# haidar-farhat/NU_Scaler

Hardware: AMD Instinct MI355X
Metric: Mpixels/sec (in+out) at 1080p→4K ×2 upscale + interp, 1/2/4/8 GPU (higher is better)
Workload: dtype u8 frames, f32 taps

## Files before the change

nu_scaler_amd/csrc/nus_host.cpp:

```cpp
#include "nus_host.hpp"

#include <condition_variable>
#include <thread>

#include "nus_copy.hpp"
#include "nus_host_util.hpp"

#include <cstdarg>
#include <cstdio>
#include <cstring>

namespace nus {


HipUpscaler::HipUpscaler(Quality q, Algorithm a) : quality_(q), algorithm_(a) {}

HipUpscaler::~HipUpscaler() { release(); }

const char *HipUpscaler::name() const
{
    switch (algorithm_) {
    case Algorithm::Bilinear: return "WgpuBilinearUpscaler";
    case Algorithm::Lanczos3: return "HipLanczos3Upscaler";
    case Algorithm::Bicubic: return "HipBicubicUpscaler";
// ... 564 lines not shown

uint32_t HipUpscaler::band_alignment(uint32_t n_frames) const
{
    switch (variant_) {
    case Variant::LanczosX2RegWin: return lanczos_x2_rows_per_wave(n_frames, false);
    case Variant::NearestX2:
    case Variant::BilinearX2Int: return 4;
    default: return 0;
    }
}

int HipUpscaler::enqueue(const uint8_t *d_in, uint8_t *d_out, uint32_t n_frames, hipStream_t stream, const BlendSrc *blend,
                         const UnitDst *unit, uint32_t row0, uint32_t rows)
{
    UpscaleLaunch L;
    L.in = d_in;
    L.out = d_out;
    L.row0 = row0;
    L.rows = rows;
    L.iw = iw_;
    L.ih = ih_;
    L.ow = ow_;
    L.oh = oh_;
    L.n_frames = n_frames;
    L.stream = stream;
    L.in_sel = input_selector(in_format_);
    if (blend) {
        L.in_stride = blend->a_stride;
        L.in_b = blend->b;
        L.in_b_stride = blend->b_stride;
        L.blend_t = blend->t;
    }
    hipEvent_t ev_begin = nullptr, ev_end = nullptr;
    if (profiling_) {
        if (prof_used_ + 2 > prof_events_.size()) {
            for (int i = 0; i < 64; ++i) {
                hipEvent_t ev;
                NUS_HIP(hipEventCreate(&ev));
                prof_events_.push_back(ev);
            }
        }
        ev_begin = prof_events_[prof_used_];
        ev_end = prof_events_[prof_used_ + 1];
        prof_used_ += 2;
        NUS_HIP(hipEventRecord(ev_begin, stream));
    }
    constexpr uint32_t kEdgeBesideMinFrames = 8;
    const bool beside = variant_ == Variant::LanczosX2RegWin && edge_stream_ && s_edge_ && ev_fork_ && ev_join_ &&
                        n_frames >= kEdgeBesideMinFrames;
    if (beside) {
        NUS_HIP(hipEventRecord(ev_fork_, stream));
        NUS_HIP(hipStreamWaitEvent(s_edge_, ev_fork_, 0));
    }
    hipError_t e = hipSuccess;
    switch (variant_) {
    case Variant::NearestTable: e = launch_nearest_table(L, dt_); break;
    case Variant::NearestX2: e = launch_nearest_x2(L); break;
    case Variant::NearestRatio: e = launch_nearest_ratio(L); break;
    case Variant::BilinearTable: e = launch_bilinear_table(L, dt_, wgsl_bilinear_); break;
    case Variant::BilinearX2Int: e = launch_bilinear_x2_int(L); break;
    case Variant::BilinearRatio: e = launch_bilinear_ratio(L, dt_); break;
    case Variant::LanczosGeneral: e = launch_lanczos_general(L, dt_, lanczos_exact_, 0); break;
    case Variant::ResizeWin:
        e = launch_resize_win(L, dt_, lanczos_exact_, resize_ncols_max_, resize_union_taps_, win_outputs_per_lane_);
        break;
    case Variant::ResizeRows:
        e = launch_resize_rows(L, dt_, lanczos_exact_, resize_ncols_max_, resize_small_taps_, resize_union_taps_);
        break;
    case Variant::ResizeDown: e = launch_resize_down(L, dt_, lanczos_exact_, resize_ncols_max_, tx_.lz_max_taps, down_seg_w_); break;
    case Variant::FsrEasu: e = launch_fsr1(L, 0, easu_sharpness(), rcas_sharpness(), fsr_fast_); break;
    case Variant::FsrRcas: e = launch_fsr1(L, 1, easu_sharpness(), rcas_sharpness()); break;
    case Variant::Fsr1Fused: e = launch_fsr1(L, 2, easu_sharpness(), rcas_sharpness(), fsr_fast_); break;
    case Variant::Fsr1TwoPass: {
        if (fsr_pending_) e = hipStreamWaitEvent(stream, ev_fsr_, 0);
        const size_t in_frame = (size_t)iw_ * ih_ * 4, out_frame = (size_t)ow_ * oh_ * 4;
        for (uint32_t done = 0; done < n_frames && e == hipSuccess; done += kFsrScratchFrames) {
            const uint32_t m = n_frames - done < kFsrScratchFrames ? n_frames - done : kFsrScratchFrames;
            UpscaleLaunch E = L;
            E.in = L.in + (size_t)done * in_frame;
            E.out = fsr_scratch_;
            E.n_frames = m;
            e = launch_fsr1(E, 0, easu_sharpness(), rcas_sharpness(), fsr_fast_);
            if (e != hipSuccess) break;
            UpscaleLaunch Rc = L;
            Rc.in = fsr_scratch_;
            Rc.out = L.out + (size_t)done * out_frame;
            Rc.iw = ow_, Rc.ih = oh_;
            Rc.n_frames = m;
            Rc.in_sel = kSelRGBA;
            e = launch_fsr1(Rc, 1, easu_sharpness(), rcas_sharpness());
        }
        if (e == hipSuccess) e = hipEventRecord(ev_fsr_, stream);
        fsr_pending_ = e == hipSuccess;
        break;
    }
    case Variant::LanczosR43RegWin: {
        uint32_t th = rows_per_wave_;
        if (th == 0) {
            const uint64_t rows_total = (uint64_t)ih_ * ((iw_ + 185) / 186) * n_frames;
            uint64_t t = rows_total / 12288;
            t = t < 12 ? 12 : (t > 36 ? 36 : t);
            const uint64_t blocks = (ih_ + t - 1) / t;
            th = (uint32_t)(((ih_ + blocks - 1) / blocks + 2) / 3 * 3);
        }
        e = launch_lanczos_r43(L, dt_, lanczos_exact_, th);
        if (e == hipSuccess) e = launch_lanczos_r43_edges(L, dt_, lanczos_exact_);
        break;
    }
    case Variant::LanczosPqRegWin: {
        uint32_t th = rows_per_wave_;
        if (th == 0) {
            const uint32_t cols = lanczos_pq_strip_cols(pq_p_, pq_q_);
            const uint64_t rows_total = (uint64_t)ih_ * ((iw_ + cols - 1) / cols) * n_frames;
            uint64_t t = rows_total / 12288;
            t = t < 12 ? 12 : (t > 36 ? 36 : t);
            const uint64_t blocks = (ih_ + t - 1) / t;
            th = (uint32_t)(((ih_ + blocks - 1) / blocks + pq_q_ - 1) / pq_q_ * pq_q_);
        }
        if (lanczos_exact_ && pq_exact_fallback_)
            e = launch_resize_win(L, dt_, true, resize_ncols_max_, resize_union_taps_, win_outputs_per_lane_);
        else
            e = launch_lanczos_pq(L, dt_, lanczos_exact_, pq_p_, pq_q_, th, pq_narrow_ && pq_narrow_allowed_);
        break;
    }
    case Variant::LanczosR32RegWin: {
        uint32_t th = rows_per_wave_;
        if (th == 0) {
            const uint64_t rows_total = (uint64_t)ih_ * ((iw_ + 239) / 240) * n_frames;
            uint64_t t = rows_total / 12288;
            t = t < 12 ? 12 : (t > 48 ? 48 : t);
            const uint64_t blocks = (ih_ + t - 1) / t;
            th = (uint32_t)((ih_ + blocks - 1) / blocks + 1) & ~1u;
        }
        e = launch_lanczos_r32(L, dt_, lanczos_exact_, th);
        if (e == hipSuccess) e = launch_lanczos_r32_edges(L, dt_, lanczos_exact_);
        break;
    }
    case Variant::LanczosXsRegWin:
    {
        uint32_t th = rows_per_wave_;
        if (th == 0) {
            const uint64_t rows_total = (uint64_t)ih_ * ((iw_ + kLanczosX2StripCols - 1) / kLanczosX2StripCols) * n_frames;
            uint64_t t = rows_total / 16384;
            t = t < 8 ? 8 : (t > 16 ? 16 : t);
            const uint64_t blocks = (ih_ + t - 1) / t;
            th = (uint32_t)((ih_ + blocks - 1) / blocks);
        }
        e = launch_lanczos_xs(L, dt_, lanczos_exact_, xs_factor_, th);
        if (e == hipSuccess) e = launch_lanczos_xs_edges(L, dt_, lanczos_exact_, xs_factor_);
        break;
    }
    case Variant::LanczosX2RegWin: {
        {
            const hipStream_t es = beside ? s_edge_ : stream;
            UpscaleLaunch E = L;
            E.stream = es;
            if (unit) {
                UpscaleLaunch R = E;
                R.in_b = nullptr;
                e = launch_lanczos_x2_edges(R, dt_, lanczos_exact_);
                if (e != hipSuccess) return fail_hip(e, "kernel launch");
                E.out = unit->out_mid;
            }
            e = launch_lanczos_x2_edges(E, dt_, lanczos_exact_);
            if (e != hipSuccess) return fail_hip(e, "kernel launch");
            if (beside) NUS_HIP(hipEventRecord(ev_join_, s_edge_));
        }
        const uint32_t th = lanczos_x2_rows_per_wave(n_frames, unit != nullptr);
        if (unit) {
            UnitOutputs U;
            U.out_mid = unit->out_mid;
            U.mid = unit->mid;
            U.order = unit_order_;
            e = launch_lanczos_x2_unit(L, dt_, lanczos_exact_, th, U);
        } else {
            e = launch_lanczos_x2(L, dt_, lanczos_exact_, th);
        }
        break;
    }
    }
    if (e != hipSuccess) {
        if (beside) (void)hipStreamSynchronize(s_edge_);
        return fail_hip(e, "kernel launch");
    }
    if (beside) NUS_HIP(hipStreamWaitEvent(stream, ev_join_, 0));
    if (ev_end) NUS_HIP(hipEventRecord(ev_end, stream));
    return kOk;
}

int HipUpscaler::set_profiling(bool on)
{
    std::lock_guard<std::mutex> lk(mu_);
    profiling_ = on;
    return kOk;
}

int HipUpscaler::profile_collect(uint64_t *launches, double *total_ms)
{
    std::lock_guard<std::mutex> lk(mu_);
    double sum = 0.0;
    if (prof_used_) NUS_HIP(hipSetDevice(device_));
    for (size_t i = 0; i + 1 < prof_used_; i += 2) {
        NUS_HIP(hipEventSynchronize(prof_events_[i + 1]));
        float ms = 0.0f;
        NUS_HIP(hipEventElapsedTime(&ms, prof_events_[i], prof_events_[i + 1]));
        sum += ms;
    }
    if (launches) *launches = prof_used_ / 2;
    if (total_ms) *total_ms = sum;
    prof_used_ = 0;
    return kOk;
}

int HipUpscaler::upscale_device(const void *d_in, void *d_out, uint32_t n_frames, hipStream_t stream)
{
    std::lock_guard<std::mutex> lk(mu_);
    if (!initialized_) return fail(kNotInitialized, "Upscaler not initialized. Call initialize() first.");
    if (!d_in || !d_out) return fail(kInvalidArgument, "upscale_device: null device pointer");
    if (n_frames == 0) return kOk;
    if ((reinterpret_cast<uintptr_t>(d_in) % 16) || (reinterpret_cast<uintptr_t>(d_out) % 16))
        return fail(kInvalidArgument, "upscale_device: device pointers must be 16-byte aligned");
    if (n_frames > 1 && (((size_t)iw_ * ih_ * 4) % 16 || ((size_t)ow_ * oh_ * 4) % 16))
        return fail(kInvalidArgument, "upscale_device: batched frames need frame sizes that are multiples of 16 bytes");
    NUS_HIP(hipSetDevice(device_));
    return enqueue(static_cast<const uint8_t *>(d_in), static_cast<uint8_t *>(d_out), n_frames, stream);
}

int HipUpscaler::upscale_blend_device(const void *d_a, size_t a_stride, const void *d_b, size_t b_stride, float t,
                                      void *d_out, uint32_t n_frames, hipStream_t stream)
{
    std::lock_guard<std::mutex> lk(mu_);
    if (!initialized_) return fail(kNotInitialized, "Upscaler not initialized. Call initialize() first.");
    if (variant_ != Variant::LanczosX2RegWin)
        return fail(kUnsupported, "upscale_blend_device: only the exact-x2 resize kernels fuse the blend; "
                                  "run interpolate + upscale separately for this configuration");
    if (!d_a || !d_b || !d_out) return fail(kInvalidArgument, "upscale_blend_device: null device pointer");
    if (n_frames == 0) return kOk;
    if ((reinterpret_cast<uintptr_t>(d_a) % 16) || (reinterpret_cast<uintptr_t>(d_b) % 16) ||
        (reinterpret_cast<uintptr_t>(d_out) % 16) || (a_stride % 16) || (b_stride % 16) ||
        (n_frames > 1 && ((size_t)ow_ * oh_ * 4) % 16))
        return fail(kInvalidArgument, "upscale_blend_device: pointers and strides must be 16-byte aligned");
    NUS_HIP(hipSetDevice(device_));
    BlendSrc bs;
    bs.b = static_cast<const uint8_t *>(d_b);
    bs.a_stride = a_stride;
    bs.b_stride = b_stride;
    bs.t = t;
    return enqueue(static_cast<const uint8_t *>(d_a), static_cast<uint8_t *>(d_out), n_frames, stream, &bs);
}

int HipUpscaler::upscale_unit_device(const void *d_a, size_t a_stride, const void *d_b, size_t b_stride, float t, void *d_mid,
                                     void *d_out_real, void *d_out_mid, uint32_t n_units, hipStream_t stream)
{
    std::lock_guard<std::mutex> lk(mu_);
    if (!initialized_) return fail(kNotInitialized, "Upscaler not initialized. Call initialize() first.");
    if (variant_ != Variant::LanczosX2RegWin)
        return fail(kUnsupported, "upscale_unit_device: only the exact-x2 resize kernels run the whole step in one launch; "
                                  "run interpolate + upscale separately for this configuration");
    if (!d_a || !d_b || !d_out_real || !d_out_mid) return fail(kInvalidArgument, "upscale_unit_device: null device pointer");
    if (!(t >= 0.0f && t <= 1.0f)) return fail(kInvalidArgument, "upscale_unit_device: t must be in [0, 1]");
    if (n_units == 0) return kOk;
    auto misaligned = [](const void *p) { return (reinterpret_cast<uintptr_t>(p) % 16) != 0; };
    if (misaligned(d_a) || misaligned(d_b) || misaligned(d_mid) || misaligned(d_out_real) || misaligned(d_out_mid) ||
        (a_stride % 16) || (b_stride % 16) ||
        (n_units > 1 && (((size_t)ow_ * oh_ * 4) % 16 || ((size_t)iw_ * ih_ * 4) % 16)))
        return fail(kInvalidArgument, "upscale_unit_device: pointers, strides and frame sizes must be multiples of 16 bytes");
    const size_t in_bytes = (size_t)iw_ * ih_ * 4;
    if ((a_stride && a_stride < in_bytes) || (b_stride && b_stride < in_bytes))
        return fail(kInvalidArgument, "upscale_unit_device: frame stride smaller than a frame");
    NUS_HIP(hipSetDevice(device_));
    BlendSrc bs;
    bs.b = static_cast<const uint8_t *>(d_b);
    bs.a_stride = a_stride ? a_stride : in_bytes;
    bs.b_stride = b_stride ? b_stride : in_bytes;
    bs.t = t;
    UnitDst ud;
    ud.out_mid = static_cast<uint8_t *>(d_out_mid);
    ud.mid = static_cast<uint8_t *>(d_mid);
    return enqueue(static_cast<const uint8_t *>(d_a), static_cast<uint8_t *>(d_out_real), n_units, stream, &bs, &ud);
}

int HipUpscaler::upscale(const uint8_t *in, size_t in_len, uint8_t *out, size_t out_cap)
{
    const uint8_t *ins[1] = {in};
    const size_t lens[1] = {in_len};
    uint8_t *outs[1] = {out};
    return upscale_batch(ins, lens, 1, outs, out_cap);
}

int HipUpscaler::ensure_streams()
{
    if (s_in_ && s_k_ && s_out_) return kOk;
    if (!s_in_) NUS_HIP(hipStreamCreateWithFlags(&s_in_, hipStreamNonBlocking));
    if (!s_k_) NUS_HIP(hipStreamCreateWithFlags(&s_k_, hipStreamNonBlocking));
    if (!s_out_) NUS_HIP(hipStreamCreateWithFlags(&s_out_, hipStreamNonBlocking));
    return kOk;
}

int HipUpscaler::ensure_slot(Slot &S, size_t in_bytes, size_t out_bytes)
{
    if (S.d_in) return kOk;
    auto make = [&]() -> int {
        NUS_HIP(hipEventCreate(&S.k_begin));
        NUS_HIP(hipEventCreate(&S.k_end));
        NUS_HIP(hipEventCreateWithFlags(&S.in_done, hipEventDisableTiming));
        NUS_HIP(hipEventCreateWithFlags(&S.out_done, hipEventDisableTiming));
        for (hipEvent_t &ev : S.chunk_done) NUS_HIP(hipEventCreateWithFlags(&ev, hipEventDisableTiming));
        for (hipEvent_t &ev : S.band_in) NUS_HIP(hipEventCreateWithFlags(&ev, hipEventDisableTiming));
        for (hipEvent_t &ev : S.band_k) NUS_HIP(hipEventCreateWithFlags(&ev, hipEventDisableTiming));
        NUS_HIP(pinned_alloc(reinterpret_cast<void **>(&S.h_in), in_bytes));
        NUS_HIP(pinned_alloc(reinterpret_cast<void **>(&S.h_out), out_bytes));
        NUS_HIP(hipMalloc(reinterpret_cast<void **>(&S.d_out), out_bytes));
        NUS_HIP(hipMalloc(reinterpret_cast<void **>(&S.d_in), in_bytes));
        return kOk;
    };
    const int rc = make();
    if (rc != kOk) release_slot(S);
// ... 497 lines not shown
```

nu_scaler_amd/csrc/nus_k_lanczos_x2.hip:

```cpp

#ifndef NUS_STORE_AUX
#define NUS_STORE_AUX 2
#endif
#include "nus_device.hpp"

namespace nus {

namespace {

struct LanczosX2Args {
    const uint8_t *in;
    const uint8_t *in_b;
    float t;
    uint32_t sel;
    uint8_t *out;
    const float *wy6;
    float wxe[6];
    float wxo[6];
    uint32_t iw, ih;
    uint32_t nstrips, nrowblocks, th;
    size_t in_frame_bytes, in_b_frame_bytes, out_frame_bytes;
    uint8_t *out_mid;
    uint8_t *mid;
    uint32_t nframes, order;
// ... 455 lines not shown
        }
        role = in_grp / A.nstrips;
        strip = in_grp % A.nstrips;
    } else {
        frame = vid / gridDim.x;
        const uint32_t wave = __builtin_amdgcn_readfirstlane((vid % gridDim.x) * 4 + (threadIdx.x >> 6));
        if (wave >= A.nstrips * A.nrowblocks) return;
        strip = wave % A.nstrips;
        rb = wave / A.nstrips + A.rb0;
    }
    const int c = (int)(strip * kLanczosX2StripCols) - 4 + lane * 4;
    int cl = c < 0 ? 0 : c;
    cl = cl > (int)A.iw - 4 ? (int)A.iw - 4 : cl;
    const uint8_t *src = A.in + (size_t)frame * A.in_frame_bytes;
    const uint8_t *src_b = BLEND ? A.in_b + (size_t)frame * A.in_b_frame_bytes : src;
    float t = A.t;
    uint8_t *out = A.out;
    MidStore ms;
    if constexpr (UNIT) {
        const bool real = role == 0;
        src_b = real ? src : src_b;
        t = real ? 0.0f : t;
        out = real ? A.out : A.out_mid;
        const bool owner = lane >= 1 && lane <= (int)(kLanczosX2StripCols / 4) && c >= 0 && c + 4 <= (int)A.iw;
        ms.lane_off = owner ? (uint32_t)c * 4u : 0x80000000u;
        ms.rs = __builtin_amdgcn_make_buffer_rsrc(A.mid + (size_t)frame * ((size_t)A.iw * A.ih * 4u), 0,
                                                  real || A.mid == nullptr ? 0u : A.iw * A.ih * 4u, 0x00020000);
    } else {
        ms.lane_off = 0;
        ms.rs = __builtin_amdgcn_make_buffer_rsrc(nullptr, 0, 0, 0x00020000);
    }
    const __amdgpu_buffer_rsrc_t rs = __builtin_amdgcn_make_buffer_rsrc(
        out + (size_t)frame * A.out_frame_bytes, 0, (uint32_t)A.out_frame_bytes, 0x00020000);
#ifndef NUS_LZ_ALIGNED_STORES
#define NUS_LZ_ALIGNED_STORES 1
#endif
#ifndef NUS_LZ_MAIN_WRITES_EDGES
#define NUS_LZ_MAIN_WRITES_EDGES 0
#endif
    auto computes_stored_pixels = [&](int L) {
        const int cc = (int)(strip * kLanczosX2StripCols) - 4 + L * 4;
#if NUS_LZ_ALIGNED_STORES && NUS_LZ_MAIN_WRITES_EDGES
        return L >= 1 && L <= (int)(kLanczosX2StripCols / 4) && cc >= 0 && cc + 4 <= (int)A.iw;
#else
        return L >= 1 && L <= (int)(kLanczosX2StripCols / 4) && cc >= 4 && cc + 8 <= (int)A.iw;
#endif
    };
    constexpr bool SWAP = lanczos_x2_swap_stores(EXACT, NARROW), LDSX = lanczos_x2_lds_exchange(EXACT, NARROW);
    RowStore st;
    st.lane = lane;
#if NUS_LZ_CONTIG_STORES
    if constexpr (SWAP) {
        const int span0 = ((int)(strip * kLanczosX2StripCols) - 4) * 8;
        const int la = lane < 32 ? lane : lane - 32, lb = lane < 32 ? lane + 32 : lane;
        const int half = lane < 32 ? 0 : 16;
        st.off_a = computes_stored_pixels(la) ? (uint32_t)(span0 + 32 * la + half) : 0x80000000u;
        st.off_b = computes_stored_pixels(lb) ? (uint32_t)(span0 + 32 * lb + half) : 0x80000000u;
        st.idx_a = st.idx_b = 0;
    } else {
        constexpr int SKIP = NUS_LZ_ALIGNED_STORES ? 32 : 0;
        const int span0 = ((int)(strip * kLanczosX2StripCols) - 4) * 8;
        const int pa = SKIP + 16 * lane, pb = SKIP + 1024 + 16 * lane;
        st.idx_a = pa / 16;
        st.idx_b = pb / 16 < 128 ? pb / 16 : 127;
        st.off_a = computes_stored_pixels(pa / 32) ? (uint32_t)(span0 + pa) : 0x80000000u;
        st.off_b = pb / 32 < 64 && computes_stored_pixels(pb / 32) ? (uint32_t)(span0 + pb) : 0x80000000u;
    }
#else
    st.off_a = computes_stored_pixels(lane) ? (uint32_t)c * 8u : 0x80000000u;
    st.off_b = st.off_a + 16u;
    st.idx_a = st.idx_b = 0;
#endif
    const uint32_t in_off = (uint32_t)cl * 4u;
    const int r0 = (int)(rb * A.th);
    const int r_end = (r0 + (int)A.th) < (int)A.ih ? (r0 + (int)A.th) : (int)A.ih;
    const int rmax = (int)A.ih - 1;
    ms.r_end = r_end;
    auto row_off = [&](int rr) {
        rr = rr < 0 ? 0 : (rr > rmax ? rmax : rr);
        return in_off + (uint32_t)rr * (A.iw * 4);
    };
    constexpr bool HIDDEN = NUS_LZ_ASM_LOADS != 0;
    constexpr int NL = BLEND ? 2 : 1;
    __shared__ u32x4 lds_rows[HIDDEN ? 4 : 1][HIDDEN ? kLzDepth * NL : 1][64];
    RowRing<BLEND> ring;
    {
        const uint32_t w = __builtin_amdgcn_readfirstlane(threadIdx.x >> 6);
        ring.slot = lds_rows[HIDDEN ? w : 0];
        ring.lds = __builtin_amdgcn_readfirstlane((uint32_t)(uintptr_t)&lds_rows[HIDDEN ? w : 0][0][0]);
        ring.lane = lane;
        st.stage = nullptr;
#if NUS_LZ_CONTIG_STORES
        if constexpr (!SWAP) {
            __shared__ u32x4 lds_stage[4][128];
            st.stage = lds_stage[w];
        }
#endif
        st.xchg = nullptr;
        if constexpr (LDSX) {
            __shared__ float lds_xchg[4][kLzXchgDwords];
            st.xchg = &lds_xchg[w][1 + lane];
        }
    }

    PhaseWeights W;
#pragma unroll
    for (int j = 0; j < 6; ++j) {
        W.e[j] = vgpr(A.wxe[j]);
        W.o[j] = vgpr(A.wxo[j]);
    }
    float win[6][16];
    AlphaRun arun;
    RowRaw<BLEND> raw[2];
    {
        RowRaw<BLEND> first[6];
#pragma unroll
        for (int j = 0; j < 6; ++j) first[j] = fetch_row_plain<BLEND>(src, src_b, row_off(r0 - 3 + j));
        if (HIDDEN) {
#pragma unroll
            for (int j = 0; j < kLzDepth; ++j) ring.request(j, src, src_b, row_off(r0 + 3 + j));
        } else {
            raw[0] = fetch_row_plain<BLEND>(src, src_b, row_off(r0 + 3));
            raw[1] = fetch_row_plain<BLEND>(src, src_b, row_off(r0 + 4));
        }
#pragma unroll
        for (int j = 0; j < 6; ++j) {
            const uint4 px = resolve_row<BLEND>(first[j], t, A.sel);
            if (!EXACT && NUS_LZ_BLEND_OPAQUE_PATH_OK(BLEND)) alpha_run_push(arun, px);
            cvt_row(px, win[j]);
            if (j >= 3) lanczos_x2_store_mid<UNIT>(px, ms, r0 - 3 + j, A.iw * 4);
        }
        if (HIDDEN) wait_vmcnt<0, 0>();
    }
    for (int rbase = r0; rbase < r_end; rbase += 6) {
#define NUS_LZ_STEP(S) \
        lanczos_x2_step<EXACT, BLEND, UNIT, S, NARROW>(win, ring, raw, arun, rbase + S, in_off, st, A, W, src, src_b, rs, t, ms); \
        if (S < 5 && rbase + S + 1 >= r_end) break
        NUS_LZ_STEP(0);
        NUS_LZ_STEP(1);
        NUS_LZ_STEP(2);
        NUS_LZ_STEP(3);
        NUS_LZ_STEP(4);
        NUS_LZ_STEP(5);
#undef NUS_LZ_STEP
    }
}

struct LanczosX2EdgeArgs {
    const uint8_t *in;
    const uint8_t *in_b;
    float t;
    uint32_t sel;
    uint8_t *out;
    const float *wy6;
    float wx[2][48];
    uint32_t iw, ih;
    size_t in_frame_bytes, in_b_frame_bytes, out_frame_bytes;
    uint32_t row0, row_end;
};

__device__ __forceinline__ uint32_t px_of(const uint4 (&row)[2], int col)
{
    const uint4 &v = row[col >> 2];
    switch (col & 3) {
    case 0: return v.x;
    case 1: return v.y;
    case 2: return v.z;
    default: return v.w;
    }
}

template <bool EXACT, int SIDE>
__device__ __forceinline__ void lanczos_x2_edge_rows(const LanczosX2EdgeArgs &A, const uint4 (&raw)[7][2], int r,
                                                     uint32_t *dst_frame)
{
    const uint32_t ow = A.iw * 2;
#pragma unroll
    for (int phase = 0; phase < 2; ++phase) {
        const uint32_t oy = 2 * (uint32_t)r + phase;
        const float *wvp = A.wy6 + (size_t)oy * 6;
        float wv[6];
#pragma unroll
        for (int j = 0; j < 6; ++j) wv[j] = wvp[j];
        float V[8][4];
#pragma unroll
        for (int col = 0; col < 8; ++col)
#pragma unroll
            for (int c = 0; c < 4; ++c) {
                float acc = ch_f32(px_of(raw[phase], col), c) * wv[0];
#pragma unroll
                for (int j = 1; j < 6; ++j) acc = mac<EXACT>(acc, ch_f32(px_of(raw[phase + j], col), c), wv[j]);
                V[col][c] = acc;
            }
        uint32_t o[8];
#pragma unroll
        for (int q = 0; q < 8; ++q) {
            const int l0 = SIDE == 0 ? (q >> 1) - 3 + (q & 1) : 1 + (q >> 1) + (q & 1);
            uint32_t px = 0;
#pragma unroll
            for (int c = 0; c < 4; ++c) {
                float acc = 0.0f;
#pragma unroll
                for (int j = 0; j < 6; ++j) {
                    int li = l0 + j;
                    li = li < 0 ? 0 : (li > 7 ? 7 : li);
                    const float w = A.wx[SIDE][q * 6 + j];
                    acc = j == 0 ? V[li][c] * w : mac<EXACT>(acc, V[li][c], w);
                }
                px = pack_u8<EXACT>(acc, c, px);
            }
            o[q] = px;
        }
        uint32_t *d = dst_frame + (size_t)oy * ow + (SIDE == 0 ? 0 : ow - 8);
        *reinterpret_cast<uint4 *>(d) = make_uint4(o[0], o[1], o[2], o[3]);
        *reinterpret_cast<uint4 *>(d + 4) = make_uint4(o[4], o[5], o[6], o[7]);
    }
}

template <bool EXACT, int BLEND>
__global__ __launch_bounds__(64) void k_lanczos3_x2_edges(const LanczosX2EdgeArgs A)
{
    const int r = (int)(A.row0 + blockIdx.x * kWave + threadIdx.x);
    if (r >= (int)A.row_end) return;
    const int side = blockIdx.y;
    const int col0 = side ? (int)A.iw - 8 : 0;
    const int rmax = (int)A.ih - 1;
    const uint8_t *src = A.in + (size_t)blockIdx.z * A.in_frame_bytes;
    const uint8_t *src_b = BLEND ? A.in_b + (size_t)blockIdx.z * A.in_b_frame_bytes : src;
    uint32_t *dst = reinterpret_cast<uint32_t *>(A.out + (size_t)blockIdx.z * A.out_frame_bytes);
    uint4 raw[7][2];
#pragma unroll
    for (int j = 0; j < 7; ++j) {
        int rr = r - 3 + j;
        rr = rr < 0 ? 0 : (rr > rmax ? rmax : rr);
        const size_t off = ((size_t)rr * A.iw + col0) * 4;
        raw[j][0] = resolve_row<BLEND>(fetch_row_plain<BLEND>(src, src_b, off), A.t, A.sel);
        raw[j][1] = resolve_row<BLEND>(fetch_row_plain<BLEND>(src, src_b, off + 16), A.t, A.sel);
    }
    if (side == 0)
        lanczos_x2_edge_rows<EXACT, 0>(A, raw, r, dst);
    else
        lanczos_x2_edge_rows<EXACT, 1>(A, raw, r, dst);
}

}

hipError_t launch_lanczos_x2(const UpscaleLaunch &L, const DeviceTables &T, bool exact, uint32_t rows_per_wave)
{
    LanczosX2Args A{};
    A.wy6 = T.lz_wy6;
    for (int j = 0; j < 6; ++j) {
        A.wxe[j] = T.lz_wxe[j];
        A.wxo[j] = T.lz_wxo[j];
    }
    A.iw = L.iw;
    A.ih = L.ih;
    A.nstrips = cdiv(L.iw, kLanczosX2StripCols);
    A.th = rows_per_wave ? rows_per_wave : 32;
    A.nrowblocks = cdiv(L.ih, A.th);
    A.rb0 = 0;
    if (L.rows) {
        if (L.row0 % A.th != 0 || L.row0 >= L.ih) return hipErrorInvalidValue;
        const uint32_t row_end = L.row0 + L.rows < L.ih ? L.row0 + L.rows : L.ih;
        if (row_end != L.ih && row_end % A.th != 0) return hipErrorInvalidValue;
        A.rb0 = L.row0 / A.th;
        A.nrowblocks = cdiv(row_end - L.row0, A.th);
    }
    A.in_frame_bytes = L.in_stride ? L.in_stride : (size_t)L.iw * L.ih * 4;
    A.in_b_frame_bytes = L.in_b_stride;
    A.out_frame_bytes = (size_t)L.ow * L.oh * 4;
    A.t = L.blend_t;
    A.sel = L.in_sel;
    const int blend = L.in_b == nullptr ? 0 : (L.blend_t == 0.5f ? 1 : 2);
#ifndef NUS_LZ_NARROW
#define NUS_LZ_NARROW 1
#endif
    const bool narrow = NUS_LZ_NARROW && blend == 0 && A.wxe[0] == 0.0f && A.wxe[5] == 0.0f && A.wxo[0] == 0.0f && A.wxo[5] == 0.0f;
    const uint32_t nwaves = A.nstrips * A.nrowblocks;
    hipError_t e = for_frame_chunks(L, [&](const uint8_t *in, uint8_t *out, uint32_t n) {
        A.in = in;
        A.in_b = L.in_b ? L.in_b + chunk_first_frame(L, in) * L.in_b_stride : nullptr;
        A.out = out;
        const dim3 block(256), grid(cdiv(nwaves, 4), n);
#define NUS_LZ(E, B) hipLaunchKernelGGL((k_lanczos3_x2<E, B, false>), grid, block, 0, L.stream, A)
        if (narrow) {
            if (exact)
                hipLaunchKernelGGL((k_lanczos3_x2<true, 0, false, true>), grid, block, 0, L.stream, A);
            else
                hipLaunchKernelGGL((k_lanczos3_x2<false, 0, false, true>), grid, block, 0, L.stream, A);
        } else if (exact) {
            if (blend == 0) NUS_LZ(true, 0); else if (blend == 1) NUS_LZ(true, 1); else NUS_LZ(true, 2);
        } else {
            if (blend == 0) NUS_LZ(false, 0); else if (blend == 1) NUS_LZ(false, 1); else NUS_LZ(false, 2);
        }
#undef NUS_LZ
    });
    return e;
}

hipError_t launch_lanczos_x2_unit(const UpscaleLaunch &L, const DeviceTables &T, bool exact, uint32_t rows_per_wave,
                                  const UnitOutputs &U)
{
    if (L.in_b == nullptr || U.out_mid == nullptr) return hipErrorInvalidValue;
    LanczosX2Args A{};
    A.wy6 = T.lz_wy6;
    for (int j = 0; j < 6; ++j) {
        A.wxe[j] = T.lz_wxe[j];
        A.wxo[j] = T.lz_wxo[j];
    }
    A.iw = L.iw;
    A.ih = L.ih;
    A.nstrips = cdiv(L.iw, kLanczosX2StripCols);
    A.th = rows_per_wave ? rows_per_wave : 32;
    A.nrowblocks = cdiv(L.ih, A.th);
    A.in_frame_bytes = L.in_stride ? L.in_stride : (size_t)L.iw * L.ih * 4;
    A.in_b_frame_bytes = L.in_b_stride;
    A.out_frame_bytes = (size_t)L.ow * L.oh * 4;
    A.t = L.blend_t;
    A.sel = L.in_sel;
    A.in = L.in;
    A.in_b = L.in_b;
    A.out = L.out;
    A.out_mid = U.out_mid;
    A.mid = U.mid;
    A.nframes = L.n_frames;
    A.order = U.order;
    const uint64_t nwaves = (uint64_t)2 * A.nstrips * A.nrowblocks * L.n_frames;
    if (nwaves / 4 + 1 >= (1ull << 31)) return hipErrorInvalidValue;
    const dim3 block(256), grid((uint32_t)((nwaves + 3) / 4));
    const bool half = L.blend_t == 0.5f;
#define NUS_LZU(E, B) hipLaunchKernelGGL((k_lanczos3_x2<E, B, true>), grid, block, 0, L.stream, A)
    if (exact) {
        if (half) NUS_LZU(true, 1); else NUS_LZU(true, 2);
    } else {
        if (half) NUS_LZU(false, 1); else NUS_LZU(false, 2);
    }
#undef NUS_LZU
    return hipGetLastError();
}

hipError_t launch_lanczos_x2_edges(const UpscaleLaunch &L, const DeviceTables &T, bool exact)
{
    LanczosX2EdgeArgs A;
    A.wy6 = T.lz_wy6;
    for (int i = 0; i < 48; ++i) {
        A.wx[0][i] = T.lz_wx_left[i];
        A.wx[1][i] = T.lz_wx_right[i];
    }
    A.iw = L.iw;
    A.ih = L.ih;
    A.in_frame_bytes = L.in_stride ? L.in_stride : (size_t)L.iw * L.ih * 4;
    A.in_b_frame_bytes = L.in_b_stride;
    A.out_frame_bytes = (size_t)L.ow * L.oh * 4;
    A.t = L.blend_t;
    A.sel = L.in_sel;
    A.row0 = L.rows ? L.row0 : 0;
    A.row_end = L.rows ? (L.row0 + L.rows < L.ih ? L.row0 + L.rows : L.ih) : L.ih;
    const int blend = L.in_b == nullptr ? 0 : (L.blend_t == 0.5f ? 1 : 2);
    return for_frame_chunks(L, [&](const uint8_t *in, uint8_t *out, uint32_t n) {
        A.in = in;
        A.in_b = L.in_b ? L.in_b + chunk_first_frame(L, in) * L.in_b_stride : nullptr;
        A.out = out;
        const dim3 block(kWave), grid(cdiv(A.row_end - A.row0, kWave), 2, n);
#define NUS_LZE(E, B) hipLaunchKernelGGL((k_lanczos3_x2_edges<E, B>), grid, block, 0, L.stream, A)
        if (exact) {
            if (blend == 0) NUS_LZE(true, 0); else if (blend == 1) NUS_LZE(true, 1); else NUS_LZE(true, 2);
        } else {
            if (blend == 0) NUS_LZE(false, 0); else if (blend == 1) NUS_LZE(false, 1); else NUS_LZE(false, 2);
        }
#undef NUS_LZE
    });
}

}
```

nu_scaler_amd/csrc/nus_kernels.hpp:

```cpp
#pragma once

#include <hip/hip_runtime.h>
#include <stddef.h>
#include <stdint.h>

namespace nus {

struct DeviceTables {
    const uint32_t *nn_sx = nullptr, *nn_sy = nullptr;
    const uint32_t *bl_x0 = nullptr, *bl_y0 = nullptr;
    const float *bl_fx = nullptr, *bl_fy = nullptr;
    const int32_t *lz_lx = nullptr, *lz_ly = nullptr;
    const uint32_t *lz_nx = nullptr, *lz_ny = nullptr;
    const float *lz_wx = nullptr, *lz_wy = nullptr;
    uint32_t lz_stride = 0;
    const uint32_t *lz_down_rows = nullptr;
    const int32_t *lz_down_done = nullptr;
    const float *lz_wy6 = nullptr;
    const float *lz_wx6 = nullptr;
    float lz_wxe[6] = {0}, lz_wxo[6] = {0};
    float lz_wx_left[48] = {0}, lz_wx_right[48] = {0};
    float lz_wxs[4][6] = {{0}};
    float lz_wxs_left[16][6] = {{0}}, lz_wxs_right[16][6] = {{0}};
    const uint32_t *lz_xs_cls_x = nullptr, *lz_xs_cls_y = nullptr;
    const float *lz_xs_wcls_x = nullptr, *lz_xs_wcls_y = nullptr;
};

constexpr uint32_t kSelRGBA = 0x03020100u, kSelBGRA = 0x03000102u;
constexpr uint32_t kSelRGBX = 0x0D020100u, kSelBGRX = 0x0D000102u;
inline uint32_t input_selector(int format)
{
    switch (format) {
    case 1: return kSelBGRA;
    case 2: return kSelRGBX;
    case 3: return kSelBGRX;
    default: return kSelRGBA;
    }
}

struct UpscaleLaunch {
    const uint8_t *in = nullptr;
    uint8_t *out = nullptr;
    uint32_t iw = 0, ih = 0, ow = 0, oh = 0;
    uint32_t n_frames = 1;
    hipStream_t stream = nullptr;
    size_t in_stride = 0;
    const uint8_t *in_b = nullptr;
    size_t in_b_stride = 0;
    float blend_t = 0.5f;
    uint32_t in_sel = kSelRGBA;
    uint32_t row0 = 0, rows = 0;
};

enum class Variant : int {
    NearestTable = 0,
    NearestX2,
    NearestRatio,
    BilinearTable,
    BilinearX2Int,
    BilinearRatio,
    LanczosGeneral,
    ResizeRows,
    ResizeWin,
    ResizeDown,
    LanczosX2RegWin,
    LanczosXsRegWin,
    LanczosR32RegWin,
    LanczosR43RegWin,
    LanczosPqRegWin,
    FsrEasu,
    FsrRcas,
    Fsr1Fused,
    Fsr1TwoPass,
};

const char *variant_name(Variant v);

hipError_t launch_nearest_table(const UpscaleLaunch &L, const DeviceTables &T);
hipError_t launch_nearest_x2(const UpscaleLaunch &L);
hipError_t launch_nearest_ratio(const UpscaleLaunch &L);
hipError_t launch_bilinear_table(const UpscaleLaunch &L, const DeviceTables &T, bool wgsl_form);
hipError_t launch_bilinear_x2_int(const UpscaleLaunch &L);
hipError_t launch_bilinear_ratio(const UpscaleLaunch &L, const DeviceTables &T);
hipError_t launch_lanczos_general(const UpscaleLaunch &L, const DeviceTables &T, bool exact,
                                  uint32_t edge_cols);
hipError_t launch_resize_rows(const UpscaleLaunch &L, const DeviceTables &T, bool exact, uint32_t ncols_max,
                              bool small_taps, uint32_t union_taps);
hipError_t launch_resize_win(const UpscaleLaunch &L, const DeviceTables &T, bool exact, uint32_t ncols_max,
                             uint32_t union_taps, uint32_t outputs_per_lane);
hipError_t launch_resize_down(const UpscaleLaunch &L, const DeviceTables &T, bool exact, uint32_t ncols_max,
                              uint32_t max_taps_x, uint32_t seg_w);
hipError_t launch_lanczos_x2(const UpscaleLaunch &L, const DeviceTables &T, bool exact,
                             uint32_t rows_per_wave);

hipError_t launch_lanczos_x2_edges(const UpscaleLaunch &L, const DeviceTables &T, bool exact);
struct UnitOutputs {
    uint8_t *out_mid = nullptr;
    uint8_t *mid = nullptr;
    uint32_t order = 1;
};
hipError_t launch_lanczos_x2_unit(const UpscaleLaunch &L, const DeviceTables &T, bool exact, uint32_t rows_per_wave,
                                  const UnitOutputs &U);
hipError_t launch_lanczos_xs(const UpscaleLaunch &L, const DeviceTables &T, bool exact, uint32_t factor,
                             uint32_t rows_per_wave);
hipError_t launch_lanczos_xs_edges(const UpscaleLaunch &L, const DeviceTables &T, bool exact, uint32_t factor);
hipError_t launch_lanczos_r32(const UpscaleLaunch &L, const DeviceTables &T, bool exact, uint32_t rows_per_wave);
hipError_t launch_lanczos_r32_edges(const UpscaleLaunch &L, const DeviceTables &T, bool exact);
hipError_t launch_lanczos_r43(const UpscaleLaunch &L, const DeviceTables &T, bool exact, uint32_t rows_per_wave);
hipError_t launch_lanczos_r43_edges(const UpscaleLaunch &L, const DeviceTables &T, bool exact);
bool lanczos_pq_supported(uint32_t P, uint32_t Q);
uint32_t lanczos_pq_strip_cols(uint32_t P, uint32_t Q);
hipError_t launch_lanczos_pq(const UpscaleLaunch &L, const DeviceTables &T, bool exact, uint32_t P, uint32_t Q, uint32_t rows_per_wave,
                             bool narrow);
hipError_t launch_fsr1(const UpscaleLaunch &L, int mode, float easu_sharpness, float rcas_sharpness, bool fast = false);

constexpr uint32_t kLanczosX2EdgeCols = 8;
#ifndef NUS_LZ_STRIP_COLS
#define NUS_LZ_STRIP_COLS 240
#endif
constexpr uint32_t kLanczosX2StripCols = NUS_LZ_STRIP_COLS;

constexpr uint32_t kInterpMaxTimes = 7;
struct TimeSet {
    float t[kInterpMaxTimes];
    uint32_t n;
};

struct WarpLaunch {
    const uint8_t *a = nullptr, *b = nullptr;
    const float *flow = nullptr;
    bool flow_half = false;
    bool fma = false;
    uint8_t *out = nullptr;
    size_t a_stride = 0, b_stride = 0;
    uint32_t w = 0, h = 0;
    float t = 0.5f;
    const float *times = nullptr;
    uint32_t n_times = 0;
    size_t out_pair_stride = 0;
    uint32_t n_pairs = 1;
    hipStream_t stream = nullptr;
    uint32_t in_sel = kSelRGBA;
};

hipError_t launch_warp_blend(const WarpLaunch &L);

hipError_t launch_swizzle_bgra(const uint8_t *in, uint8_t *out, size_t npx, hipStream_t stream);

hipError_t launch_rgba8_to_f32(const uint8_t *in, float *out, uint32_t w, uint32_t h, hipStream_t stream);
hipError_t launch_blur(const float *in, float *out, uint32_t w, uint32_t h, bool horizontal, hipStream_t stream);
hipError_t launch_downsample(const float *in, float *out, uint32_t w, uint32_t h, hipStream_t stream);
hipError_t launch_horn_schunck(const float *i1, const float *i2, const float *flow_in, float *flow_out, uint32_t w,
                               uint32_t h, float lambda, hipStream_t stream);
struct FlowImages {
    uint32_t w = 0, h = 0;
    uint32_t n = 1;
    hipStream_t stream = nullptr;
};
enum JacobiKernel { kJacobiAuto = 0, kJacobiTiles = 1, kJacobiStream = 2, kJacobiStreamFast = 3 };
struct PyramidLevelLaunch {
    FlowImages img;
    const void *in = nullptr;
    bool u8_input = false;
    float *level_lum = nullptr;
    float *next = nullptr;
    size_t in_stride = 0;
    size_t lum_stride = 0, next_stride = 0;
};
hipError_t launch_pyramid_level(const PyramidLevelLaunch &L, int kernel);
hipError_t launch_pyramid_level_fast(const PyramidLevelLaunch &L);
struct HsPrepareLaunch {
    FlowImages img;
    const float *i1 = nullptr, *i2 = nullptr;
    bool luminance_planes = false;
    float *coef = nullptr;
    size_t img_stride = 0, coef_stride = 0;
};
hipError_t launch_hs_prepare(const HsPrepareLaunch &L);
struct HsCoarseFlow {
    const float *flow = nullptr;
    uint32_t w = 0, h = 0;
    float scale = 0.0f;
    size_t stride = 0;
};
hipError_t launch_hs_level_setup(const HsPrepareLaunch &L, const HsCoarseFlow &coarse, float *flow, size_t flow_stride);
struct HsWarp {
    const uint8_t *frames = nullptr;
    size_t frame_stride = 0;
    uint8_t *mid = nullptr;
    float t = 0.5f;
    uint32_t sel = 0;
    uint32_t out_half = 0;
    uint32_t in_half = 0;
};
hipError_t launch_flow_to_half(const float *src, void *dst, size_t n_cells, hipStream_t stream);
struct HsIterateLaunch {
    FlowImages img;
    const float *coef = nullptr;
    const float *lum1 = nullptr;
    size_t coef_stride = 0, lum_stride = 0;
    float lambda = 0.0f;
    uint32_t iterations = 0;
    bool zero_start = false;
    float *flow_a = nullptr, *flow_b = nullptr;
    float *final_out = nullptr;
    size_t flow_stride = 0, final_stride = 0;
    int kernel = kJacobiAuto;
    HsCoarseFlow coarse;
    const HsWarp *warp = nullptr;
};
struct HsIterateResult {
    float *flow = nullptr, *spare = nullptr;
    bool warped = false, wrote_half = false;
};
hipError_t launch_hs_iterate(const HsIterateLaunch &L, HsIterateResult *result);
bool hs_iterate_streams(uint32_t w, uint32_t h, uint32_t n, int kernel);
hipError_t launch_flow_upsample(const FlowImages &D, const HsCoarseFlow &coarse, float *dst, size_t dst_stride);

constexpr uint32_t kProbeValuBlocks = 2048;
hipError_t launch_probe(int kind, const void *d_src, void *d_dst, size_t bytes, uint32_t iters, hipStream_t stream);

constexpr uint32_t kMetricsBlock = 256;
struct MetricsShape {
    uint32_t sse_blocks = 0, ssim_blocks = 0;
    uint32_t tiles_x = 0, tiles_y = 0;
    size_t sse_offset = 0, ssim_offset = 0, workspace_bytes = 0;
};
MetricsShape metrics_shape(uint32_t w, uint32_t h, uint32_t frames, bool mse, bool ssim);
hipError_t launch_metrics(const uint8_t *a, size_t a_stride, const uint8_t *b, size_t b_stride, uint32_t w, uint32_t h,
                          uint32_t frames, bool mse, bool ssim, void *workspace, double *out, hipStream_t stream);

constexpr uint32_t kBmRunPixels = 64;
constexpr uint32_t kBmMaxRadius = 24;
struct BmShape {
    uint32_t blocks_x = 0, blocks_y = 0, runs_x = 0, rough_groups = 0;
    size_t rough_offset = 0, workspace_bytes = 0;
    size_t g_offset = 0, sad_g_offset = 0, sad_f_offset = 0, chosen_offset = 0, state_offset = 0;
};
constexpr uint32_t kBmMaxTolerance = 96;
BmShape bm_shape(uint32_t w, uint32_t h, uint32_t bs, uint32_t n_pairs, bool bidir = false);
size_t bm_lds_bytes(uint32_t bs, uint32_t R);
struct BmLaunch {
    const uint8_t *a = nullptr, *b = nullptr;
    size_t a_stride = 0, b_stride = 0;
    uint32_t w = 0, h = 0, n_pairs = 1;
    uint32_t bs = 16, R = 16;
    const uint16_t *rank = nullptr, *cand = nullptr;
    void *workspace = nullptr;
// ... 60 lines not shown
```

Baseline: 1.551 million.

## Share edge rows via LDS and merge real/interp edge launches into one

The Lanczos x2 edge kernel now has each lane load a single input row into LDS, so neighbouring lanes reuse it instead of each lane fetching seven rows. The vertical weights are loaded as vectors, and the horizontal taps skip clamped duplicates. The separate real-frame and interpolated-frame edge launches in unit mode are merged into one launch with a doubled grid y-dimension. The cost is 6 halo lanes per wave that only load, plus a wave barrier. This code only handles the border columns, so its effect on the whole pipeline is small.

```diff
diff --git a/nu_scaler_amd/csrc/nus_host.cpp b/nu_scaler_amd/csrc/nus_host.cpp
--- a/nu_scaler_amd/csrc/nus_host.cpp
+++ b/nu_scaler_amd/csrc/nus_host.cpp
@@ -740,17 +740,9 @@
     }
     case Variant::LanczosX2RegWin: {
         {
-            const hipStream_t es = beside ? s_edge_ : stream;
             UpscaleLaunch E = L;
-            E.stream = es;
-            if (unit) {
-                UpscaleLaunch R = E;
-                R.in_b = nullptr;
-                e = launch_lanczos_x2_edges(R, dt_, lanczos_exact_);
-                if (e != hipSuccess) return fail_hip(e, "kernel launch");
-                E.out = unit->out_mid;
-            }
-            e = launch_lanczos_x2_edges(E, dt_, lanczos_exact_);
+            E.stream = beside ? s_edge_ : stream;
+            e = launch_lanczos_x2_edges(E, dt_, lanczos_exact_, unit ? unit->out_mid : nullptr);
             if (e != hipSuccess) return fail_hip(e, "kernel launch");
             if (beside) NUS_HIP(hipEventRecord(ev_join_, s_edge_));
         }
diff --git a/nu_scaler_amd/csrc/nus_k_lanczos_x2.hip b/nu_scaler_amd/csrc/nus_k_lanczos_x2.hip
--- a/nu_scaler_amd/csrc/nus_k_lanczos_x2.hip
+++ b/nu_scaler_amd/csrc/nus_k_lanczos_x2.hip
@@ -631,6 +631,7 @@
     float t;
     uint32_t sel;
     uint8_t *out;
+    uint8_t *out_mid;
     const float *wy6;
     float wx[2][48];
     uint32_t iw, ih;
@@ -638,57 +639,43 @@
     uint32_t row0, row_end;
 };
 
-__device__ __forceinline__ uint32_t px_of(const uint4 (&row)[2], int col)
-{
-    const uint4 &v = row[col >> 2];
-    switch (col & 3) {
-    case 0: return v.x;
-    case 1: return v.y;
-    case 2: return v.z;
-    default: return v.w;
-    }
-}
+constexpr int kLzEdgeRun = kWave - 6;
+
+typedef float f32x4_a4 __attribute__((ext_vector_type(4), aligned(4)));
 
 template <bool EXACT, int SIDE>
-__device__ __forceinline__ void lanczos_x2_edge_rows(const LanczosX2EdgeArgs &A, const uint4 (&raw)[7][2], int r,
-                                                     uint32_t *dst_frame)
+__device__ __forceinline__ void lanczos_x2_edge_rows(const LanczosX2EdgeArgs &A, const uint32_t *plane, const float (&wv)[12],
+                                                     int r, uint32_t *dst_frame)
 {
     const uint32_t ow = A.iw * 2;
 #pragma unroll
     for (int phase = 0; phase < 2; ++phase) {
         const uint32_t oy = 2 * (uint32_t)r + phase;
-        const float *wvp = A.wy6 + (size_t)oy * 6;
-        float wv[6];
-#pragma unroll
-        for (int j = 0; j < 6; ++j) wv[j] = wvp[j];
         float V[8][4];
 #pragma unroll
-        for (int col = 0; col < 8; ++col)
-#pragma unroll
-            for (int c = 0; c < 4; ++c) {
-                float acc = ch_f32(px_of(raw[phase], col), c) * wv[0];
-#pragma unroll
-                for (int j = 1; j < 6; ++j) acc = mac<EXACT>(acc, ch_f32(px_of(raw[phase + j], col), c), wv[j]);
-                V[col][c] = acc;
+        for (int j = 0; j < 6; ++j) {
+#pragma unroll
+            for (int col = 0; col < 8; ++col) {
+                const uint32_t px = plane[col * kWave + phase + j];
+#pragma unroll
+                for (int c = 0; c < 4; ++c)
+                    V[col][c] = j == 0 ? ch_f32(px, c) * wv[phase * 6] : mac<EXACT>(V[col][c], ch_f32(px, c), wv[phase * 6 + j]);
             }
-        uint32_t o[8];
-#pragma unroll
-        for (int q = 0; q < 8; ++q) {
-            const int l0 = SIDE == 0 ? (q >> 1) - 3 + (q & 1) : 1 + (q >> 1) + (q & 1);
-            uint32_t px = 0;
-#pragma unroll
-            for (int c = 0; c < 4; ++c) {
-                float acc = 0.0f;
-#pragma unroll
-                for (int j = 0; j < 6; ++j) {
-                    int li = l0 + j;
-                    li = li < 0 ? 0 : (li > 7 ? 7 : li);
-                    const float w = A.wx[SIDE][q * 6 + j];
-                    acc = j == 0 ? V[li][c] * w : mac<EXACT>(acc, V[li][c], w);
-                }
-                px = pack_u8<EXACT>(acc, c, px);
+            __builtin_amdgcn_sched_barrier(0);
+        }
+        uint32_t o[8] = {0, 0, 0, 0, 0, 0, 0, 0};
+#pragma unroll
+        for (int c = 0; c < 4; ++c) {
+#pragma unroll
+            for (int q = 0; q < 8; ++q) {
+                const int l0 = SIDE == 0 ? (q >> 1) - 3 + (q & 1) : 1 + (q >> 1) + (q & 1);
+                const int j0 = l0 < 0 ? -l0 : 0, j1 = l0 + 5 > 7 ? 8 - l0 : 6;
+                float acc = V[l0 + j0][c] * A.wx[SIDE][q * 6 + j0];
+#pragma unroll
+                for (int j = j0 + 1; j < j1; ++j) acc = mac<EXACT>(acc, V[l0 + j][c], A.wx[SIDE][q * 6 + j]);
+                o[q] = pack_u8<EXACT>(acc, c, o[q]);
             }
-            o[q] = px;
+            __builtin_amdgcn_sched_barrier(0);
         }
         uint32_t *d = dst_frame + (size_t)oy * ow + (SIDE == 0 ? 0 : ow - 8);
         *reinterpret_cast<uint4 *>(d) = make_uint4(o[0], o[1], o[2], o[3]);
@@ -697,29 +684,53 @@
 }
 
 template <bool EXACT, int BLEND>
-__global__ __launch_bounds__(64) void k_lanczos3_x2_edges(const LanczosX2EdgeArgs A)
-{
-    const int r = (int)(A.row0 + blockIdx.x * kWave + threadIdx.x);
-    if (r >= (int)A.row_end) return;
-    const int side = blockIdx.y;
+__global__ __launch_bounds__(kWave) void k_lanczos3_x2_edges(const LanczosX2EdgeArgs A)
+{
+    __shared__ uint32_t lds_patch[8 * kWave];
+    const int lane = (int)threadIdx.x;
+    const int r = (int)(A.row0 + blockIdx.x * kLzEdgeRun) - 3 + lane;
+    const int side = blockIdx.y & 1;
     const int col0 = side ? (int)A.iw - 8 : 0;
     const int rmax = (int)A.ih - 1;
+    const int rc = r < 0 ? 0 : (r > rmax ? rmax : r);
     const uint8_t *src = A.in + (size_t)blockIdx.z * A.in_frame_bytes;
     const uint8_t *src_b = BLEND ? A.in_b + (size_t)blockIdx.z * A.in_b_frame_bytes : src;
-    uint32_t *dst = reinterpret_cast<uint32_t *>(A.out + (size_t)blockIdx.z * A.out_frame_bytes);
-    uint4 raw[7][2];
-#pragma unroll
-    for (int j = 0; j < 7; ++j) {
-        int rr = r - 3 + j;
-        rr = rr < 0 ? 0 : (rr > rmax ? rmax : rr);
-        const size_t off = ((size_t)rr * A.iw + col0) * 4;
-        raw[j][0] = resolve_row<BLEND>(fetch_row_plain<BLEND>(src, src_b, off), A.t, A.sel);
-        raw[j][1] = resolve_row<BLEND>(fetch_row_plain<BLEND>(src, src_b, off + 16), A.t, A.sel);
-    }
+    uint8_t *out = A.out;
+    float t = A.t;
+    if constexpr (BLEND != 0) {
+        if (A.out_mid != nullptr) {
+            const bool real = (blockIdx.y >> 1) == 0;
+            src_b = real ? src : src_b;
+            t = real ? 0.0f : t;
+            out = real ? A.out : A.out_mid;
+        }
+    }
+    const size_t off = ((size_t)rc * A.iw + col0) * 4;
+    const RowRaw<BLEND> lo = fetch_row_plain<BLEND>(src, src_b, off), hi = fetch_row_plain<BLEND>(src, src_b, off + 16);
+    float wv[12];
+    {
+        const f32x4_a4 *wp = reinterpret_cast<const f32x4_a4 *>(A.wy6 + (size_t)rc * 12);
+#pragma unroll
+        for (int k = 0; k < 3; ++k) {
+            const f32x4_a4 w = wp[k];
+            wv[4 * k] = w.x, wv[4 * k + 1] = w.y, wv[4 * k + 2] = w.z, wv[4 * k + 3] = w.w;
+        }
+    }
+    {
+        const uint4 p0 = resolve_row<BLEND>(lo, t, A.sel), p1 = resolve_row<BLEND>(hi, t, A.sel);
+        uint32_t *mine = lds_patch + lane;
+        mine[0 * kWave] = p0.x, mine[1 * kWave] = p0.y, mine[2 * kWave] = p0.z, mine[3 * kWave] = p0.w;
+        mine[4 * kWave] = p1.x, mine[5 * kWave] = p1.y, mine[6 * kWave] = p1.z, mine[7 * kWave] = p1.w;
+    }
+    __builtin_amdgcn_fence(__ATOMIC_RELEASE, "wavefront");
+    __builtin_amdgcn_wave_barrier();
+    __builtin_amdgcn_fence(__ATOMIC_ACQUIRE, "wavefront");
+    if (lane < 3 || lane >= 3 + kLzEdgeRun || r >= (int)A.row_end) return;
+    uint32_t *dst = reinterpret_cast<uint32_t *>(out + (size_t)blockIdx.z * A.out_frame_bytes);
     if (side == 0)
-        lanczos_x2_edge_rows<EXACT, 0>(A, raw, r, dst);
+        lanczos_x2_edge_rows<EXACT, 0>(A, lds_patch + lane - 3, wv, r, dst);
     else
-        lanczos_x2_edge_rows<EXACT, 1>(A, raw, r, dst);
+        lanczos_x2_edge_rows<EXACT, 1>(A, lds_patch + lane - 3, wv, r, dst);
 }
 
 }
@@ -818,8 +829,9 @@
     return hipGetLastError();
 }
 
-hipError_t launch_lanczos_x2_edges(const UpscaleLaunch &L, const DeviceTables &T, bool exact)
-{
+hipError_t launch_lanczos_x2_edges(const UpscaleLaunch &L, const DeviceTables &T, bool exact, uint8_t *out_mid)
+{
+    if (out_mid != nullptr && L.in_b == nullptr) return hipErrorInvalidValue;
     LanczosX2EdgeArgs A;
     A.wy6 = T.lz_wy6;
     for (int i = 0; i < 48; ++i) {
@@ -835,12 +847,15 @@
     A.sel = L.in_sel;
     A.row0 = L.rows ? L.row0 : 0;
     A.row_end = L.rows ? (L.row0 + L.rows < L.ih ? L.row0 + L.rows : L.ih) : L.ih;
+    if (A.row0 >= A.row_end) return hipErrorInvalidValue;
     const int blend = L.in_b == nullptr ? 0 : (L.blend_t == 0.5f ? 1 : 2);
     return for_frame_chunks(L, [&](const uint8_t *in, uint8_t *out, uint32_t n) {
+        const size_t first = chunk_first_frame(L, in);
         A.in = in;
-        A.in_b = L.in_b ? L.in_b + chunk_first_frame(L, in) * L.in_b_stride : nullptr;
+        A.in_b = L.in_b ? L.in_b + first * L.in_b_stride : nullptr;
         A.out = out;
-        const dim3 block(kWave), grid(cdiv(A.row_end - A.row0, kWave), 2, n);
+        A.out_mid = out_mid ? out_mid + first * A.out_frame_bytes : nullptr;
+        const dim3 block(kWave), grid(cdiv(A.row_end - A.row0, kLzEdgeRun), out_mid ? 4 : 2, n);
 #define NUS_LZE(E, B) hipLaunchKernelGGL((k_lanczos3_x2_edges<E, B>), grid, block, 0, L.stream, A)
         if (exact) {
             if (blend == 0) NUS_LZE(true, 0); else if (blend == 1) NUS_LZE(true, 1); else NUS_LZE(true, 2);
diff --git a/nu_scaler_amd/csrc/nus_kernels.hpp b/nu_scaler_amd/csrc/nus_kernels.hpp
--- a/nu_scaler_amd/csrc/nus_kernels.hpp
+++ b/nu_scaler_amd/csrc/nus_kernels.hpp
@@ -93,7 +93,7 @@
 hipError_t launch_lanczos_x2(const UpscaleLaunch &L, const DeviceTables &T, bool exact,
                              uint32_t rows_per_wave);
 
-hipError_t launch_lanczos_x2_edges(const UpscaleLaunch &L, const DeviceTables &T, bool exact);
+hipError_t launch_lanczos_x2_edges(const UpscaleLaunch &L, const DeviceTables &T, bool exact, uint8_t *out_mid = nullptr);
 struct UnitOutputs {
     uint8_t *out_mid = nullptr;
     uint8_t *mid = nullptr;
```

After: 1.447 million. 0.933x the previous value.
